# Funatiq/cuclark

Hardware: AMD Instinct MI355X
Metric: Mreads/sec (10M x 150bp, k=31) (higher is better)
Workload: dtype u64

## Files before the change

cuclark_amd/csrc/mic_kernels.hip:

```cpp
#include "mic_internal.h"
#include "mic_device.h"
#include "mic_ksketch.h"
#include "mic_hitmap.h"
#include "mic_join2.h"

#include <stdlib.h>
#include <type_traits>

#ifndef MIC_EXP
#define MIC_EXP 0
#endif
#ifndef MIC_FUNNEL64
#define MIC_FUNNEL64 1
#endif
#ifndef MIC_X
#define MIC_X 0
#endif
#if MIC_X & 8
__device__ unsigned long long g_entry_walk[3];
extern "C" int mic_debug_entry_walk(unsigned long long out[3], int reset) {
  if (hipMemcpyFromSymbol(out, HIP_SYMBOL(g_entry_walk), sizeof(g_entry_walk)) != hipSuccess) return -1;
  const unsigned long long z[3] = {0, 0, 0};
  if (reset && hipMemcpyToSymbol(HIP_SYMBOL(g_entry_walk), z, sizeof(z)) != hipSuccess) return -1;
  return 0;
// ... 931 lines not shown
              bool more0 = v0 && e0 < 6, more1 = v1 && e1 < 6;
              uint32_t hit0 = 0, hit1 = 0;
              e0 = e0 < 5 ? e0 : 5; e1 = e1 < 5 ? e1 : 5;
              for (;;) {
                const uint32_t g0 = q0[e0], g1 = q1[e1];
                const uint32_t a0 = q0[6 + 3 * e0], b0 = q0[7 + 3 * e0], c0 = q0[8 + 3 * e0], p0 = q0[24 + e0];
                const uint32_t a1 = q1[6 + 3 * e1], b1 = q1[7 + 3 * e1], c1 = q1[8 + 3 * e1], p1 = q1[24 + e1];
                const bool same0 = more0 && g0 == t0, same1 = more1 && g1 == t1;
                const bool m0 = same0 && ((p0 >> (16 + (w - 1) - ao[0])) & 1) && s_extract(a0, b0, c0, (int)ao[0], k) == ko[0];
                const bool m1 = same1 && ((p1 >> (16 + (w - 1) - ao[1])) & 1) && s_extract(a1, b1, c1, (int)ao[1], k) == ko[1];
                if (m0) hit0 = (p0 & 0xFFFFu) + 1;
                if (m1) hit1 = (p1 & 0xFFFFu) + 1;
                {
                  const bool cr0 = same0 && (p0 >> 16) == 0, cr1 = same1 && (p1 >> 16) == 0;
                  if (__ballot(cr0) | __ballot(cr1)) {
                    uint64_t kp = (uint64_t)__builtin_amdgcn_kernarg_segment_ptr();
                    asm volatile("" : "+s"(kp));
                    const __attribute__((address_space(4))) MicQueryArgs* kc = (const __attribute__((address_space(4))) MicQueryArgs*)kp;
                    const uint4* side = kc->t.side; const uint32_t smask = kc->t.side_mask;
                    const uint64_t mm = (1ULL << (2 * m)) - 1;
                    if (side && cr0 && s_extract(a0, b0, c0, w - 1, m) == ((ko[0] >> (2 * ao[0])) & mm)) hit0 = s_side_probe(side, smask, ko[0]);
                    if (side && cr1 && s_extract(a1, b1, c1, w - 1, m) == ((ko[1] >> (2 * ao[1])) & mm)) hit1 = s_side_probe(side, smask, ko[1]);
                  }
                }
                more0 = same0 && !m0 && e0 < 5; more1 = same1 && !m1 && e1 < 5;
                e0 += more0 ? 1u : 0u; e1 += more1 ? 1u : 0u;
                if (!(__ballot(more0) | __ballot(more1))) break;
              }
              if (v0) { o0_ = hit0; y0_ = 0xFFFFFFFFu; }
              if (v1) { o1_ = hit1; y1_ = 0xFFFFFFFFu; }
              const bool n0 = v0 && !hit0 && (mz0 & MIC_S_NEXT), n1 = v1 && !hit1 && (mz1 & MIC_S_NEXT);
              if (__ballot(n0) | __ballot(n1)) {
                if (n0 && q0[5] <= t0) y0_ = q0[31];
                if (n1 && q1[5] <= t1) y1_ = q1[31];
              }
            }
          }
        };
        while (__ballot(sl0 != 0xFFFFFFFFu) | __ballot(sl1 != 0xFFFFFFFFu)) {
          uint32_t nx0, nx1;
          level(sl0, sl1, res0, res1, nx0, nx1);
          sl0 = nx0; sl1 = nx1;
        }
        tally2(res0, res1, acc, n_ent, overflow, total, lane);
      }
    }
    uint32_t t_hdr, t_pp, t_pe;
    asm volatile("s_waitcnt vmcnt(0)" ::: "memory");
    __builtin_amdgcn_wave_barrier();
    ahead_take(ahead_sel ? ahead1 : ahead0, n_pp, t_hdr, t_pp, t_pe);
    __builtin_amdgcn_wave_barrier();
    {
      uint64_t kp = (uint64_t)__builtin_amdgcn_kernarg_segment_ptr();
      asm volatile("" : "+s"(kp));
      const __attribute__((address_space(4))) MicQueryArgs* kc = (const __attribute__((address_space(4))) MicQueryArgs*)kp;
      struct { uint32_t* results; uint32_t* rows; uint32_t* flagged; uint32_t row_words, flagged_cap; } fa;
      fa.results = kc->results; fa.rows = kc->rows; fa.flagged = kc->flagged; fa.row_words = kc->row_words; fa.flagged_cap = kc->flagged_cap;
      finish_read(acc, n_ent, total, overflow, r, fa, lane);
    }
    ahead_issue(ahead_sel ? ahead0 : ahead1, t_pp, r + 3 * n_waves);
    ahead_sel ^= 1;
    cur_pp = n_pp; cur_pe = n_pe; cur_hdr = t_hdr; n_pp = t_pp; n_pe = t_pe;
  }
}


__device__ __forceinline__ uint64_t wballot(bool p) { return __builtin_amdgcn_ballot_w64(p); }
#if defined(__has_builtin) && __has_builtin(__builtin_amdgcn_writelane)
__device__ __forceinline__ int mic_writelane(int value, int lane, int old) { return __builtin_amdgcn_writelane(value, lane, old); }
#else
extern "C" __device__ int mic_writelane(int value, int lane, int old) __asm("llvm.amdgcn.writelane.i32");
#endif

static_assert(MIC_RMAX <= 32, "tally_counts sums the first two rows of lanes");
#define MIC_R_CROWDED (-16)
__device__ __forceinline__ void tally_counts(uint32_t lab1, uint32_t cnt, RowAcc& acc, uint32_t& n_ent, uint32_t& overflow,
                                             uint32_t& total, int lane) {
  uint64_t mm = wballot(lab1 != 0);
  while (mm) {
    const uint32_t l1 = __builtin_amdgcn_readlane(lab1, __builtin_ctzll(mm));
    const bool mine = lab1 == l1;
    mm &= ~wballot(mine);
    const uint32_t c = mine ? cnt : 0u;
    uint32_t sum = 0;
    {
      uint32_t v = c;
      v += (uint32_t)__builtin_amdgcn_update_dpp(0, (int)v, 0x111, 0xF, 0xF, true);
      v += (uint32_t)__builtin_amdgcn_update_dpp(0, (int)v, 0x112, 0xF, 0xF, true);
      v += (uint32_t)__builtin_amdgcn_update_dpp(0, (int)v, 0x114, 0xF, 0xF, true);
      v += (uint32_t)__builtin_amdgcn_update_dpp(0, (int)v, 0x118, 0xF, 0xF, true);
      sum = __builtin_amdgcn_readlane(v, 15) + __builtin_amdgcn_readlane(v, 31);
    }
    total += sum;
    if (wballot(acc.label1 == l1)) {
      if (acc.label1 == l1) acc.count += sum;
    } else if (n_ent < 64) {
      acc.label1 = (uint32_t)mic_writelane((int)l1, (int)n_ent, (int)acc.label1);
      acc.count = (uint32_t)mic_writelane((int)sum, (int)n_ent, (int)acc.count);
      ++n_ent;
    } else {
      overflow = 1;
    }
  }
}

template <int KK, int MM, bool FWD, bool PART>
__global__ void __launch_bounds__(64 * MIC_M_WPB, 32 / MIC_M_WPB) query_kernel_r(const MicQueryArgs a) {
  __shared__ uint4 s_stage[MIC_M_WPB][MIC_RMAX * MIC_MSTRIDE + (MIC_RMAX / 8 - 1) * MIC_R_SKEW];
  __shared__ uint16_t s_rec[MIC_M_WPB][132];
  __shared__ uint32_t s_ahead[MIC_M_WPB][2][64];
  __shared__ uint32_t s_part[PART ? MIC_M_WPB : 1][2];
  const int lane = threadIdx.x & 63;
  const int wv = __builtin_amdgcn_readfirstlane(threadIdx.x >> 6);
  uint4* stage = s_stage[wv];
  uint16_t* rec = s_rec[wv];
  const uint32_t wave0 = __builtin_amdgcn_readfirstlane(blockIdx.x * MIC_M_WPB + wv);
  const uint32_t n_waves = gridDim.x * MIC_M_WPB;
  const MicTable& t = a.t;
  if (PART) { if (lane == 0) { s_part[wv][0] = t.slot_lo; s_part[wv][1] = t.slot_cnt; } __builtin_amdgcn_wave_barrier(); }
  const int k = KK ? KK : t.k, m = MM ? MM : t.m, ctx = k - m;
  const uint4* __restrict__ slots = t.slots;
  const uint16_t* __restrict__ cont = a.cont;
  auto below = [](uint64_t mask) { return (uint32_t)__builtin_amdgcn_mbcnt_hi((uint32_t)(mask >> 32), __builtin_amdgcn_mbcnt_lo((uint32_t)mask, 0u)); };

  uint32_t* ahead0 = s_ahead[wv][0];
  uint32_t* ahead1 = s_ahead[wv][1];
  auto lane_copy = [&]() { int ln = lane; asm volatile("" : "+v"(ln)); return ln; };
  auto ahead_issue = [&](uint32_t* entry, uint32_t pp_w, uint32_t r_ptr, const int ln) {
    const uint64_t abase = ((uint64_t)(cont + pp_w)) & ~3ULL;
    const uint32_t rr = r_ptr < a.n_reads ? r_ptr : a.n_reads - 1;
    const uint64_t pbase = (uint64_t)(a.reads_ptr + rr) - 48;
    if (ln < 12)
      __builtin_amdgcn_global_load_lds((const __attribute__((address_space(1))) void*)((const uint32_t*)abase + lane),
                                       (__attribute__((address_space(3))) void*)entry, 4, 0, 0);
    uint64_t pb = pbase + 48;
    asm volatile("" : "+s"(pb));
    if (ln < 2)
      __builtin_amdgcn_global_load_lds((const __attribute__((address_space(1))) void*)((const uint32_t*)pb + lane),
                                       (__attribute__((address_space(3))) void*)(entry + 12), 4, 0, 0);
  };
  auto ahead_take = [&](const uint32_t* entry, uint32_t pp_w, uint32_t& hdr, uint32_t& npp, uint32_t& npe) {
    const uint32_t raw = entry[lane];
    npp = __builtin_amdgcn_readlane(raw, 12); npe = __builtin_amdgcn_readlane(raw, 13);
    const bool odd = (((uint64_t)(cont + pp_w)) >> 1) & 1;
    const uint32_t first = __builtin_amdgcn_readfirstlane(raw);
    hdr = odd ? first >> 16 : first & 0xFFFFu;
  };
  auto ahead_word = [&](const uint32_t* entry, uint32_t pp_w) {
    const uint32_t raw = entry[lane];
    const bool odd = (((uint64_t)(cont + pp_w)) >> 1) & 1;
    const uint32_t up = (uint32_t)__builtin_amdgcn_update_dpp(0, (int)raw, 0x101, 0xF, 0xF, true);
    return __builtin_amdgcn_perm(up, raw, odd ? 0x05040706u : 0x03020504u);
  };
  uint32_t cur_pp, cur_pe, cur_hdr, n_pp, n_pe, ahead_sel;
  {
    const uint32_t r0 = wave0 < a.n_reads ? wave0 : a.n_reads - 1;
    cur_pp = __builtin_amdgcn_readfirstlane(a.reads_ptr[r0]); cur_pe = __builtin_amdgcn_readfirstlane(a.reads_ptr[r0 + 1]);
    ahead_issue(ahead0, cur_pp, wave0 + n_waves, lane_copy());
    asm volatile("s_waitcnt vmcnt(0)" ::: "memory");
    __builtin_amdgcn_wave_barrier();
    ahead_take(ahead0, cur_pp, cur_hdr, n_pp, n_pe);
    ahead_issue(ahead1, n_pp, wave0 + 2 * n_waves, lane_copy());
    ahead_sel = 1;
  }
  constexpr bool PIPE = KK != 0 && (MIC_R_PIPE >= 2 || (MIC_R_PIPE == 1 && FWD));
  struct Round {
    uint32_t G0, G1, G2, cur;
    int jmax, jmin, remaining;
  };
  struct NoGap {};
  struct Gap { uint32_t len1, b2, g0; };
  auto front = [&](const uint32_t first, const uint32_t cend, const uint32_t base, const uint32_t nk, const bool use_ahead, uint32_t& wd_out,
                   const auto gp) __attribute__((always_inline)) -> uint32_t {
    constexpr bool GAP = std::is_same<decltype(gp), const Gap>::value;
    int ln = lane;
    asm volatile("" : "+v"(ln));
    uint32_t wd;
    if constexpr (GAP) {
      const uint32_t* entry = ahead_sel ? ahead0 : ahead1;
      const uint32_t j = (uint32_t)ln < 12u ? (uint32_t)ln : 0u;
      const uint32_t d = j2_dword(j, gp.len1, gp.b2);
      wd = j2_window(ahead_word(entry, cur_pp), entry[d], entry[d + 1u], j, gp.len1, gp.b2);
    } else {
      wd = use_ahead ? ahead_word(ahead_sel ? ahead0 : ahead1, cur_pp)
                     : window_word_w(cont, first, cend, base, ln, false, 0u);
    }
    wd_out = wd;
    const uint32_t n_act = nk - base < 128u ? nk - base : 128u;
    if constexpr (KK == F3_K && MM == F3_M) {
      uint32_t p0, s0, s1, s2, q0, q1, q2;
      if constexpr (GAP) sampled_positions3<!FWD, true>(wd, lane, n_act, p0, s0, s1, s2, q0, q1, q2, gp.len1, gp.g0);
      else sampled_positions3<!FWD>(wd, lane, n_act, p0, s0, s1, s2, q0, q1, q2);
      const uint32_t pv = (uint32_t)__builtin_amdgcn_update_dpp(-1, (int)q2, 0x138, 0xF, 0xF, false);
      const bool f0 = q0 != pv, f1 = q1 != q0, f2 = q2 != q1;
      const uint64_t b0 = wballot(f0), b1 = wballot(f1), b2 = wballot(f2);
      const uint32_t R = __popcll(b0) + __popcll(b1) + __popcll(b2) - 1u;
      uint32_t c = __builtin_amdgcn_mbcnt_hi((uint32_t)(b0 >> 32), __builtin_amdgcn_mbcnt_lo((uint32_t)b0, 0u));
      c = __builtin_amdgcn_mbcnt_hi((uint32_t)(b1 >> 32), __builtin_amdgcn_mbcnt_lo((uint32_t)b1, c));
      c = __builtin_amdgcn_mbcnt_hi((uint32_t)(b2 >> 32), __builtin_amdgcn_mbcnt_lo((uint32_t)b2, c));
      __builtin_amdgcn_wave_barrier();
      const uint32_t c1 = c + (f0 ? 1u : 0u), c2 = c1 + (f1 ? 1u : 0u);
      if (f0) rec[c] = f3_record(s0, p0);
      if (f1) rec[c1] = f3_record(s1, p0 + 1u);
      if (f2) rec[c2] = f3_record(s2, p0 + 2u);
      __builtin_amdgcn_wave_barrier();
      return R;
    }
    const bool past = n_act + (uint32_t)(k - s_tlen(k, m)) >= 129u;
    uint32_t qa0, qa1;
    if constexpr (GAP) sampled_positions<!FWD, true>(wd, ln, lane, k, m, past, qa0, qa1, gp.len1);
    else sampled_positions<!FWD>(wd, ln, lane, k, m, past, qa0, qa1);
    qa0 = (uint32_t)lane < n_act ? qa0 : 0xFFu;
    qa1 = 64u + (uint32_t)lane < n_act ? qa1 : 0xFFu;
    if constexpr (GAP) {
      qa0 = (uint32_t)lane - gp.g0 >= (uint32_t)(k - 1) ? qa0 : 0xFFu;
      qa1 = 64u + (uint32_t)lane - gp.g0 >= (uint32_t)(k - 1) ? qa1 : 0xFFu;
    }
    const uint32_t last0 = __builtin_amdgcn_readlane(qa0, 63);
    uint32_t p0 = (uint32_t)__builtin_amdgcn_update_dpp(-1, (int)qa0, 0x138, 0xF, 0xF, false);
    uint32_t p1 = (uint32_t)__builtin_amdgcn_update_dpp((int)last0, (int)qa1, 0x138, 0xF, 0xF, false);
    const bool f0 = qa0 != p0, f1 = qa1 != p1;
    const uint64_t b0 = wballot(f0), b1 = wballot(f1);
    const uint32_t R0 = __popcll(b0), R = R0 + __popcll(b1) - (n_act < 128u ? 1u : 0u);
    __builtin_amdgcn_wave_barrier();
    if (f0) rec[below(b0)] = (uint16_t)(qa0 | ((uint32_t)lane << 8));
    if (f1) rec[R0 + below(b1)] = (uint16_t)(qa1 | ((64u + (uint32_t)lane) << 8));
    if (__builtin_expect(n_act == 128u, 0)) {
      asm volatile("" ::: "memory");
      if (ln == 0) rec[R] = (uint16_t)(128u << 8);
    }
    __builtin_amdgcn_wave_barrier();
    return R;
  };
  const uint32_t xsh = (64u - 2u * (uint32_t)k) & 31u;
  auto region_x = [&](uint32_t A0, uint32_t A1, uint32_t& lo, uint32_t& hi) {
    if (k > 16) {
      lo = __builtin_amdgcn_alignbit(A0, A1, xsh) & (m >= 16 ? 0xFFFFFFFFu : (1u << ((2 * m) & 31)) - 1u);
      hi = m > 16 ? (A0 >> xsh) & ((1u << ((2 * m - 32) & 31)) - 1u) : 0u;
    } else {
      const uint64_t x = ((((uint64_t)A0 << 32) | A1) << (2 * ctx)) >> (64 - 2 * m);
      lo = (uint32_t)x; hi = (uint32_t)(x >> 32);
    }
  };
  auto setup = [&](const uint32_t wd, const uint32_t rbase, const uint32_t R, Round& L, uint32_t& nrun_out, const auto gp) __attribute__((always_inline)) {
    constexpr bool GAP = std::is_same<decltype(gp), const Gap>::value;
    const uint32_t nrun = R - rbase < MIC_RMAX ? R - rbase : MIC_RMAX;
    nrun_out = nrun;
    bool vr = (uint32_t)lane < nrun;
    const uint32_t ri = vr ? rbase + (uint32_t)lane : 0u;
    const uint32_t rc0 = rec[ri], rc1 = rec[ri + 1];
    const int qa = (int)(rc0 & 255u), i0 = (int)(rc0 >> 8);
    if constexpr (GAP) vr = vr && (uint32_t)i0 != gp.g0;
    const int n = (int)(rc1 >> 8) - i0;
    const int s1 = qa - ctx - 1;
    const int D = s1 >> 4;
    const uint32_t tsh = 30u - 2u * (uint32_t)(s1 & 15);
    const int a0 = D << 2;
    const uint32_t W0 = (uint32_t)__builtin_amdgcn_ds_bpermute(a0, (int)wd), W1 = (uint32_t)__builtin_amdgcn_ds_bpermute(a0 + 4, (int)wd),
                   W2 = (uint32_t)__builtin_amdgcn_ds_bpermute(a0 + 8, (int)wd), W3 = (uint32_t)__builtin_amdgcn_ds_bpermute(a0 + 12, (int)wd);
    uint32_t G0 = __builtin_amdgcn_alignbit(W0, W1, tsh), G1 = __builtin_amdgcn_alignbit(W1, W2, tsh), G2 = __builtin_amdgcn_alignbit(W2, W3, tsh);
    uint32_t key, xhi;
    region_x(G0, G1, key, xhi);
    bool rev = false;
    if (!FWD) {
      const uint32_t sh = 96u - 2u * (uint32_t)(k + ctx);
      const uint32_t r0 = __builtin_bitreverse32(G2), r1 = __builtin_bitreverse32(G1), r2 = __builtin_bitreverse32(G0);
      uint32_t q0, q1, q2;
      if (KK != 0 && sh != 0) {
        q0 = swap_comp_pairs(__builtin_amdgcn_alignbit(r0, r1, 33u - sh), __builtin_amdgcn_alignbit(r0, r1, 31u - sh));
        q1 = swap_comp_pairs(__builtin_amdgcn_alignbit(r1, r2, 33u - sh), __builtin_amdgcn_alignbit(r1, r2, 31u - sh));
        q2 = swap_comp_pairs(r2 << (sh - 1u), r2 << (sh + 1u));
      } else {
        q0 = sh ? __builtin_amdgcn_alignbit(r0, r1, 32u - sh) : r0;
        q1 = sh ? __builtin_amdgcn_alignbit(r1, r2, 32u - sh) : r1;
        q2 = r2 << sh;
        q0 = swap_comp_pairs(q0 >> 1, q0 << 1); q1 = swap_comp_pairs(q1 >> 1, q1 << 1); q2 = swap_comp_pairs(q2 >> 1, q2 << 1);
      }
      uint32_t kr, hr;
      region_x(q0, q1, kr, hr);
      rev = hr < xhi || (hr == xhi && kr < key);
      G0 = rev ? q0 : G0; G1 = rev ? q1 : G1; G2 = rev ? q2 : G2;
      key = rev ? kr : key; xhi = rev ? hr : xhi;
    }
    const int jmaxf = qa - i0, jminf = jmaxf - n + 1;
    const int jmax = rev ? ctx - jminf : jmaxf, jmin = rev ? ctx - jmaxf : jminf;
    uint32_t cur = vr ? sslot_of_x32(key, xhi, (uint32_t)t.n_main) : 0xFFFFFFFFu;
    bool mine = vr;
    if (PART) {
      mine = vr && cur - s_part[wv][0] < s_part[wv][1];
      cur = mine ? cur : 0xFFFFFFFFu;
    }
    L.G0 = G0; L.G1 = G1; L.G2 = G2; L.cur = cur;
    L.jmax = jmax; L.jmin = jmin; L.remaining = mine ? n : 0;
  };
  auto issue = [&](const uint32_t cur, const uint32_t nrun, const int ln) __attribute__((always_inline)) {
    uint32_t sidx[MIC_RMAX / 8];
    __builtin_amdgcn_wave_barrier();
    if (ln < MIC_RMAX) ((uint32_t*)stage)[lane] = cur;
    __builtin_amdgcn_wave_barrier();
    uint32_t so = (uint32_t)(uintptr_t)(__attribute__((address_space(3))) void*)stage;
    asm volatile("" : "+s"(so));
#pragma unroll
    for (int i = 0; i < MIC_RMAX / 8; ++i) sidx[i] = ((const uint32_t*)stage)[8 * i + (lane >> 3)];
#pragma unroll
    for (int i = 0; i < MIC_RMAX / 8; ++i) {
      if (8u * i >= nrun) break;
      if (sidx[i] != 0xFFFFFFFFu)
        __builtin_amdgcn_global_load_lds((const __attribute__((address_space(1))) void*)(slots + (uint64_t)sidx[i] * 8 + (lane & 7)),
                                         (__attribute__((address_space(3))) void*)(uintptr_t)(so + 16u * (64 + MIC_R_SKEW) * (uint32_t)i), 16, 0, 0);
    }
  };
  auto consume = [&](Round& L, RowAcc& acc, uint32_t& n_ent, uint32_t& overflow, uint32_t& total, uint32_t& cg) __attribute__((always_inline)) {
    const uint32_t G0 = L.G0, G1 = L.G1, G2 = L.G2;
    uint32_t key, xhi_;
    region_x(G0, G1, key, xhi_);
    const int jmax = L.jmax, jmin = L.jmin;
    uint32_t cur = L.cur;
    int remaining = L.remaining;
    for (;;) {
      asm volatile("s_waitcnt vmcnt(0)" ::: "memory");
      __builtin_amdgcn_wave_barrier();
      const bool vl = cur != 0xFFFFFFFFu;
      const uint32_t* q = (const uint32_t*)(stage + (vl ? staged_at((uint32_t)lane) : 0));
      const uint4 ka = *(const uint4*)q;
      const uint2 kb = *(const uint2*)(q + 4);
      uint32_t e = (ka.x < key) + (ka.y < key) + (ka.z < key) + (ka.w < key) + (kb.x < key) + (kb.y < key);
      const uint32_t mz = q[30];
      const uint64_t m_vl = wballot(vl);
      uint64_t m_more = m_vl & wballot(e < 6), m_pos = 0;
      e = e < 5 ? e : 5;
#if MIC_X & 8
      uint32_t ew_pass = 0;
#endif
      for (;;) {
        uint32_t e3 = e + (e << 1);
        asm volatile("" : "+v"(e3));
        uint32_t g = q[e], g1 = q[e + 1], S0 = q[6 + e3], S1 = q[7 + e3], S2 = q[8 + e3], pl = q[24 + e];
        asm volatile("" : "+v"(S2));
        const uint64_t m_same = m_more & wballot(g == key);
        const uint64_t m_next = wballot(g1 == key);
        const uint32_t d0 = G0 ^ S0, d1 = G1 ^ S1, d2 = G2 ^ S2;
        const uint64_t m_hit = m_same & (k > 16
                                             ? wballot(((d0 & ((1u << ((32 - 2 * ctx) & 31)) - 1u)) | (d1 >> xsh)) == 0)
                                             : wballot((((((uint64_t)d0 << 32) | d1) << (2 * ctx)) >> (64 - 2 * m)) == 0));
        const uint32_t dl = d0 >> (32 - 2 * ctx);
        const uint32_t dr = k > 16 ? __builtin_amdgcn_alignbit(d1, d2, xsh)
                                        : (uint32_t)((((((uint64_t)d0 << 32) | d1)) << ((2 * k) & 63)) >> 32);
        const int left = __builtin_ctz(dl | (1u << (2 * ctx))) >> 1;
        const int right = __builtin_clz(dr | (1u << (31 - 2 * ctx))) >> 1;
        const int hi = left < jmax ? left : jmax, lo = ctx - right > jmin ? ctx - right : jmin;
        const uint32_t range = ((2u << (hi & 31)) - 1u) & (~0u << (lo & 31));
        const uint32_t hits = __builtin_amdgcn_inverse_ballot_w64(m_hit) ? (uint32_t)__popc((pl >> 16) & range) : 0u;
#if MIC_X & 8
        const bool ew_hit = wballot(hits != 0) != 0;
        if (lane == 0 && ew_pass < 2u) atomicAdd(&g_entry_walk[ew_pass], 1ull);
        if (lane == 0 && ew_pass == 1u && ew_hit) atomicAdd(&g_entry_walk[2], 1ull);
        ++ew_pass;
#endif
        const uint32_t lab_new = (pl & 0xFFFFu) + 1u;
#if !(MIC_X & 16)
        tally_counts(hits ? lab_new : 0u, hits, acc, n_ent, overflow, total, lane);
#endif
#if MIC_X & 32
        break;
#endif
#if !(MIC_X & 1)
        remaining = __builtin_amdgcn_inverse_ballot_w64(m_hit & wballot(pl < 0x10000u)) ? MIC_R_CROWDED : remaining;
#endif
        remaining -= (int)hits;
        m_pos = wballot(remaining > 0);
        m_more = m_same & m_pos & wballot(e < 5);
#if !(MIC_X & 256)
        m_more &= m_next;
#endif
        e += __builtin_amdgcn_inverse_ballot_w64(m_more) ? 1u : 0u;
        if (!m_more) break;
      }
#if MIC_X & 64
      break;
#endif
      const uint64_t m_nx = m_pos & wballot((mz & MIC_S_NEXT) != 0);
      if (!m_nx) break;
      cur = 0xFFFFFFFFu;
      if (__builtin_amdgcn_inverse_ballot_w64(m_nx) && q[5] <= key) cur = q[31];
      if (!wballot(cur != 0xFFFFFFFFu)) break;
      remaining = (cur == 0xFFFFFFFFu && remaining > 0) ? 0 : remaining;
      issue(cur, MIC_RMAX, lane_copy());
    }
    if (!(MIC_X & 2) && __builtin_expect(wballot(remaining <= MIC_R_CROWDED) != 0, 0)) {
      const bool crowded = remaining <= MIC_R_CROWDED;
      const uint32_t n_c = (uint32_t)__popcll(wballot(crowded));
      uint64_t kpv = (uint64_t)__builtin_amdgcn_kernarg_segment_ptr();
      asm volatile("" : "+v"(kpv));
      const MicQueryArgs* kv = (const MicQueryArgs*)kpv;
      uint32_t* cw = kv->crowd;
      uint32_t* itb = kv->crowd_items;
      const uint32_t icap = kv->crowd_item_cap;
      uint32_t ib = 0xFFFFFFFFu;
      if (cw != nullptr && cg != MIC_CG_DENSE) {
        uint32_t v = 0;
        if (lane == 0) v = atomicAdd(&cw[1], n_c);
        ib = __builtin_amdgcn_readfirstlane(v);
      }
      asm volatile("" : "+v"(ib));
      const bool room = ib <= icap && n_c <= icap - ib;
      if (crowded && room) {
        uint32_t* it = itb + 8 * ((size_t)ib + below(wballot(crowded)));
        it[0] = G0; it[1] = G1; it[2] = G2; it[3] = (uint32_t)jmin | ((uint32_t)jmax << 8);
        it[4] = cg;
      }
      cg = __builtin_amdgcn_readfirstlane(room ? (ib | ((n_c - 1u) << 27)) : MIC_CG_DENSE);
    }
  };
  auto finish = [&](const RowAcc& acc, uint32_t n_ent, uint32_t total, uint32_t overflow, uint32_t r, const uint32_t cg) __attribute__((always_inline)) {
    uint32_t spilled = 0;
    if (!(MIC_X & 4) && __builtin_expect(cg != MIC_CG_NONE, 0)) {
      uint64_t kpv = (uint64_t)__builtin_amdgcn_kernarg_segment_ptr();
      asm volatile("" : "+v"(kpv));
      const MicQueryArgs* kv = (const MicQueryArgs*)kpv;
      uint32_t* cw = kv->crowd;
      uint32_t* pool = kv->crowd_pool;
      const uint32_t pcap = kv->crowd_pend_cap, wcap = kv->crowd_pool_cap;
      uint32_t p = 0xFFFFFFFFu, off = 0;
      if (cg != MIC_CG_DENSE) {
        if (lane == 0) { p = atomicAdd(&cw[0], 1u); off = atomicAdd(&cw[2], 2u * n_ent); }
        p = __builtin_amdgcn_readfirstlane(p); off = __builtin_amdgcn_readfirstlane(off);
      }
      asm volatile("" : "+v"(p), "+v"(off));
      const bool room = off <= wcap && 2u * n_ent <= wcap - off;
      if (p < pcap) {
        uint32_t* pd = cw + MIC_CROWD_HDR + 8 * (size_t)p;
        if (lane == 0) { pd[0] = r; pd[1] = total; pd[2] = room ? (n_ent | (overflow << 8)) : 0xFFFFFFFFu; pd[3] = off; pd[4] = cg; }
        if (room && (uint32_t)lane < n_ent) { uint32_t* pe_ = pool + (size_t)off + 2 * lane; pe_[0] = acc.label1; pe_[1] = acc.count; }
      }
      spilled = __builtin_amdgcn_readfirstlane((p < pcap && room) ? 1u : 0u);
      if (!spilled) {
        if (lane == 0 && cw != nullptr && cg != MIC_CG_DENSE) atomicAdd(&cw[3], 1u);
        overflow = 1;
      }
    }
    if (!spilled) {
      uint64_t kp = (uint64_t)__builtin_amdgcn_kernarg_segment_ptr();
      asm volatile("" : "+s"(kp));
      const __attribute__((address_space(4))) MicQueryArgs* kc = (const __attribute__((address_space(4))) MicQueryArgs*)kp;
      struct { uint32_t* results; uint32_t* rows; uint32_t* flagged; uint32_t row_words, flagged_cap; } fa;
      fa.results = kc->results; fa.rows = kc->rows; fa.flagged = kc->flagged; fa.row_words = kc->row_words; fa.flagged_cap = kc->flagged_cap;
      finish_read(acc, n_ent, total, overflow, r, fa, lane);
    }
  };

  uint32_t r = wave0; bool p_valid = false;
  auto step = [&](Round& P, Round& N) __attribute__((always_inline)) -> bool {
    const bool have = r < a.n_reads;
    uint32_t pp = cur_pp;
    const uint32_t pe = cur_pe;
    bool shape = false, simple = false;
    uint32_t n_nrun = 0, plen0 = 0, pp1 = 0;
    uint32_t slot2 = J2_NONE;
    if (have) {
      plen0 = cur_hdr; pp1 = pp + 1 + (plen0 + 7) / 8;
      shape = plen0 - (uint32_t)k < 128u && pp1 == pe;
      if (!shape && plen0 - (uint32_t)k < 128u && pp1 < pe) {
        const uint32_t rel = pp1 - cur_pp + (uint32_t)((((uint64_t)(cont + cur_pp)) >> 1) & 1);
        if (rel < 24u) {
          const uint32_t v = (ahead_sel ? ahead0 : ahead1)[rel >> 1];
          slot2 = __builtin_amdgcn_readfirstlane((rel & 1u) ? v >> 16 : v & 0xFFFFu);
          shape = slot2 == 0;
        }
      }
      uint32_t n_wd = 0, R = MIC_RMAX + 1u, g0 = 0xFFFFFFFFu;
      if (PIPE && shape) {
        R = front(pp + 1, pp1, 0u, plen0 - (uint32_t)k + 1u, true, n_wd, NoGap{});
      } else if constexpr (PIPE) {
        const uint32_t odd = (uint32_t)((((uint64_t)(cont + cur_pp)) >> 1) & 1);
        const uint32_t* entry = ahead_sel ? ahead0 : ahead1;
        const J2Shape j2 = j2_shape(plen0, slot2, pe - pp, odd, (uint32_t)k,
                                    [&](uint32_t u) { return (uint32_t)__builtin_amdgcn_readfirstlane(j2_half(entry[u >> 1], u)); });
        if (__builtin_expect(j2.ok != 0u, 0)) {
          R = front(pp + 1, pp1, 0u, j2.n_act, true, n_wd, Gap{j2.len1, j2.b2, j2.g0});
          g0 = j2.g0;
        }
      }
      if (PIPE && R <= MIC_RMAX) { setup(n_wd, 0u, R, N, n_nrun, Gap{0u, 0u, g0}); simple = true; }
    }
    if (PIPE && p_valid) {
      RowAcc acc; acc.label1 = 0; acc.count = 0;
      uint32_t n_ent = 0, overflow = 0, total = 0, cg = MIC_CG_NONE;
      consume(P, acc, n_ent, overflow, total, cg);
      finish(acc, n_ent, total, overflow, r - n_waves, cg);
    } else {
      asm volatile("s_waitcnt vmcnt(0)" ::: "memory");
    }
    if (!have) return false;
    if (!simple) {
      RowAcc acc; acc.label1 = 0; acc.count = 0;
      uint32_t n_ent = 0, overflow = 0, total = 0, cg = MIC_CG_NONE;
      auto chunk = [&](const uint32_t first, const uint32_t cend, const uint32_t base, const uint32_t nk, const bool use_ahead) __attribute__((always_inline)) {
        uint32_t wd;
        const uint32_t R = front(first, cend, base, nk, use_ahead, wd, NoGap{});
        for (uint32_t rbase = 0; rbase < R; rbase += MIC_RMAX) {
          Round L; uint32_t nrun;
          setup(wd, rbase, R, L, nrun, NoGap{});
          issue(L.cur, nrun, lane_copy());
          consume(L, acc, n_ent, overflow, total, cg);
        }
      };
      if (!PIPE && shape) chunk(pp + 1, pp1, 0u, plen0 - (uint32_t)k + 1u, true);
      else {
        bool first_part = true;
        while (pp < pe) {
          uint32_t plen;
          {
            const uint32_t rel = pp - cur_pp + (uint32_t)((((uint64_t)(cont + cur_pp)) >> 1) & 1);
            if (first_part) plen = cur_hdr;
            else if (rel < 24u) {
              const uint32_t v = (ahead_sel ? ahead0 : ahead1)[rel >> 1];
              plen = __builtin_amdgcn_readfirstlane((rel & 1u) ? v >> 16 : v & 0xFFFFu);
            } else plen = __builtin_amdgcn_readfirstlane((uint32_t)cont[pp]);
          }
          const bool ahead_ok = first_part;
          first_part = false;
          if (plen == 0) break;
          const uint32_t first = pp + 1;
          pp = first + (plen + 7) / 8;
          if (plen < (uint32_t)k) continue;
          const uint32_t nk = plen - k + 1;
          const uint32_t cend = pp;
          for (uint32_t base = 0; base < nk; base += 128) chunk(first, cend, base, nk, ahead_ok && base == 0);
        }
      }
      finish(acc, n_ent, total, overflow, r, cg);
    }
    uint32_t t_hdr, t_pp, t_pe;
    __builtin_amdgcn_wave_barrier();
    ahead_take(ahead_sel ? ahead1 : ahead0, n_pp, t_hdr, t_pp, t_pe);
    __builtin_amdgcn_wave_barrier();
    const int ln = lane_copy();
    ahead_issue(ahead_sel ? ahead0 : ahead1, t_pp, r + 3 * n_waves, ln);
    ahead_sel ^= 1;
    cur_pp = n_pp; cur_pe = n_pe; cur_hdr = t_hdr; n_pp = t_pp; n_pe = t_pe;
    p_valid = simple;
    if (simple) issue(N.cur, n_nrun, ln);
    r += n_waves;
    return true;
  };
  Round Ra, Rb;
  while (step(Ra, Rb) && step(Rb, Ra)) {}
}

__global__ void __launch_bounds__(256) crowd_finish_kernel(const MicQueryArgs a) {
  const int lane = threadIdx.x & 63;
  const uint32_t wave0 = __builtin_amdgcn_readfirstlane(blockIdx.x * 4 + (threadIdx.x >> 6)), n_waves = gridDim.x * 4;
  const uint32_t* __restrict__ cw = a.crowd;
  const uint32_t pcap = a.crowd_pend_cap;
  uint32_t np = cw[0];
  np = np < pcap ? np : pcap;
  const uint32_t* __restrict__ pend = cw + MIC_CROWD_HDR;
  const uint32_t* __restrict__ items = a.crowd_items;
  const uint32_t* __restrict__ pool = a.crowd_pool;
  const uint4* __restrict__ side = a.t.side;
  const uint32_t smask = a.t.side_mask;
  const int k = a.t.k, ctx = k - a.t.m;
  for (uint32_t p = wave0; p < np; p += n_waves) {
    const uint4 h = *(const uint4*)(pend + 8 * (size_t)p);
    const uint32_t r = __builtin_amdgcn_readfirstlane(h.x), meta = __builtin_amdgcn_readfirstlane(h.z), off = __builtin_amdgcn_readfirstlane(h.w);
    uint32_t total = __builtin_amdgcn_readfirstlane(h.y);
    uint32_t g = __builtin_amdgcn_readfirstlane(pend[8 * (size_t)p + 4]);
    if (meta == 0xFFFFFFFFu) continue;
    uint32_t n_ent = meta & 0xFFu, overflow = (meta >> 8) & 1u;
    RowAcc acc; acc.label1 = 0; acc.count = 0;
    if ((uint32_t)lane < n_ent) { const uint2 e = *(const uint2*)(pool + off + 2 * lane); acc.label1 = e.x; acc.count = e.y; }
    while (g != MIC_CG_NONE) {
      const uint32_t ib = g & 0x7FFFFFFu, n_c = (g >> 27) + 1u;
      g = __builtin_amdgcn_readfirstlane(items[8 * (size_t)ib + 4]);
      for (uint32_t b = 0; b < n_c; b += 4) {
        const uint32_t idx = b + ((uint32_t)lane >> 4);
        const bool valid = idx < n_c;
        uint4 it = make_uint4(0, 0, 0, 0);
        if (valid) it = *(const uint4*)(items + 8 * (size_t)(ib + idx));
        const int jmin = (int)(it.w & 0xFFu), jmax = (int)((it.w >> 8) & 0xFFu);
        int j = jmin + (lane & 15);
        bool go = valid && j <= jmax;
        j = go ? j : jmin;
        const uint64_t K = s_extract(it.x, it.y, it.z, ctx - j, k);
        uint32_t hsh = s_side_hash(K, smask), got = 0;
        while (wballot(go)) {
          uint4 c = make_uint4(0, 0, 0, 0);
          if (go) c = load_slot_quarter(side + hsh);
          if (go) {
            if (c.z == 0) go = false;
            else if (c.x == (uint32_t)K && c.y == (uint32_t)(K >> 32)) { got = c.z; go = false; }
            else hsh = (hsh + 1) & smask;
          }
        }
        tally2(got, 0u, acc, n_ent, overflow, total, lane);
      }
    }
    finish_read(acc, n_ent, total, overflow, r, a, lane);
  }
}


__global__ void merge_rows_kernel(const uint32_t* __restrict__ ra, const uint32_t* __restrict__ rb,
                                  uint32_t* __restrict__ out, uint32_t row_words, size_t n,
                                  uint32_t* __restrict__ results) {
  size_t i = (size_t)blockIdx.x * blockDim.x + threadIdx.x;
  if (i >= n) return;
  const uint32_t* a = ra + i * row_words; const uint32_t* b = rb + i * row_words; uint32_t* o = out + i * row_words;
  uint32_t na = a[0], nb = b[0], ia = 0, ib = 0, no = 0;
  bool ok = na != MIC_ROW_INVALID && nb != MIC_ROW_INVALID;
  if (!ok) { na = 0; nb = 0; }
  while (ia < na || ib < nb) {
    uint32_t va = ia < na ? a[1 + ia] : 0xFFFFFFFFu, vb = ib < nb ? b[1 + ib] : 0xFFFFFFFFu;
    uint32_t ta = ia < na ? (va & 0xFFFF) : 0x10000u, tb = ib < nb ? (vb & 0xFFFF) : 0x10000u;
    uint32_t tgt, cnt;
    if (ta < tb) { tgt = ta; cnt = va >> 16; ++ia; }
    else if (tb < ta) { tgt = tb; cnt = vb >> 16; ++ib; }
    else { tgt = ta; cnt = (va >> 16) + (vb >> 16); ++ia; ++ib; }
    if (no + 1 < row_words && cnt <= 0xFFFF) o[1 + no] = (cnt << 16) | tgt; else ok = false;
    ++no;
  }
  o[0] = ok ? no : MIC_ROW_INVALID;
  (void)results;
}

__global__ void result_rows_kernel(const uint32_t* __restrict__ rows, uint32_t row_words,
                                   uint32_t* __restrict__ results, size_t n) {
  size_t i = (size_t)blockIdx.x * blockDim.x + threadIdx.x;
  if (i >= n) return;
  const uint32_t* row = rows + i * row_words;
  uint32_t cnt = row[0], sum = 0, best = 0, ib = 0, sb = 0, is = 0, flags = 0;
  if (cnt == MIC_ROW_INVALID) { cnt = 0; flags = MIC_FLAG_ROW_OVERFLOW_; }
  for (uint32_t e = 0; e < cnt; ++e) {
    uint32_t v = row[1 + e], tgt = v & 0xFFFF, sc = v >> 16;
    if (sc > best) { sb = best; is = ib; best = sc; ib = tgt + 1; }
    else if (sc > sb) { sb = sc; is = tgt + 1; }
    sum += sc;
  }
  uint4* out = (uint4*)(results + i * 8);
  out[0] = make_uint4(sum, ib, best, is);
  out[1] = make_uint4(sb, cnt, flags, 0);
}

template <bool KEY64>
__device__ inline uint32_t probe_scalar(const MicTable& t, uint64_t kmer) {
  constexpr uint32_t CAP = KEY64 ? MIC_CAP64 : MIC_CAP32;
  uint64_t c = canonical(kmer, t.k);
  uint64_t q = mic_div(c, t.div);
  uint64_t rem = c - q * t.div.d;
  if (rem < t.shard_start || rem >= t.shard_end) return 0;
  if (!KEY64 && (q >> 32) != 0) return 0;
  uint64_t slot = rem - t.shard_start;
  for (;;) {
    uint4 qq[4];
#pragma unroll
    for (int j = 0; j < 4; ++j) qq[j] = t.slots[slot * 4 + j];
    uint32_t n = qq[0].w & 0xFF;
    uint64_t lastk = 0;
#pragma unroll
    for (int j = 0; j < 4; ++j) {
      uint32_t m = match_quarter<KEY64>(qq[j], (uint32_t)q, (uint32_t)(q >> 32), j);
      if (m) return m;
    }
    lastk = KEY64 ? (((uint64_t)qq[3].y << 32) | qq[3].x) : (uint64_t)qq[3].y;
    if (n <= CAP || q <= lastk) return 0;
    slot = (uint64_t)(qq[0].w >> 8) | ((uint64_t)(qq[1].w >> 8) << 24);
  }
}

__device__ inline uint32_t probe_scalar_m(const MicTable& t, uint64_t kmer) {
  uint64_t c = canonical(kmer, t.k);
  if (t.sharded) {
    uint64_t q = mic_div(c, t.div);
    uint64_t rem = c - q * t.div.d;
    if (rem < t.shard_start || rem >= t.shard_end) return 0;
  }
  uint64_t slot = mslot_of_kmer(kmer, t.k, t.m, (uint32_t)t.n_main);
  for (;;) {
    const uint4* q = t.slots + slot * 8;
    const uint4 meta = q[7];
    const uint32_t n = MIC_M_N(meta.z);
    uint32_t cnt = 0;
    bool eq = false;
    for (uint32_t e = 0; e < n; ++e) {
      uint4 kv = q[e >> 1];
      uint64_t key = (e & 1) ? (((uint64_t)kv.w << 32) | kv.z) : (((uint64_t)kv.y << 32) | kv.x);
      if (key <= c) { ++cnt; eq = key == c; }
    }
    if (!(meta.z & MIC_M_DIR)) {
      if (!eq) return 0;
      const uint32_t e = cnt - 1;
      uint4 lw = q[6 + (e >> 3)];
      uint32_t wi = (e & 7) >> 1;
      uint32_t word = wi == 0 ? lw.x : wi == 1 ? lw.y : wi == 2 ? lw.z : lw.w;
      return ((e & 1) ? (word >> 16) : (word & 0xFFFF)) + 1;
    }
    if (cnt == 0) return 0;
    slot = (uint64_t)q[6].x + (cnt - 1);
  }
}
// ... 452 lines not shown
```

Before: 2285.

## Restructure read pipeline loop into steady-state fast path with fallback road

Replaces the single generic step lambda, which carried have/simple/p_valid flags every iteration, with a split control flow. A steady-state loop alternates the take_up/back_half/issue halves while reads stay simple, and falls back to a plain per-read path when they do not. The ahead-buffer selection flag becomes swapped pointers (e_cur/e_nxt) instead of ternaries on each access. The goal is to cut scalar branching and selects in the hot loop and to let the compiler schedule the pipelined path more tightly. It adds code size and more complex loop exits, which risks register pressure or a missed final drain.

Result: faster. 2323 (median of 6 runs) (+1.7%).

```diff
diff --git a/cuclark_amd/csrc/mic_kernels.hip b/cuclark_amd/csrc/mic_kernels.hip
--- a/cuclark_amd/csrc/mic_kernels.hip
+++ b/cuclark_amd/csrc/mic_kernels.hip
@@ -1107,7 +1107,7 @@
     const uint32_t up = (uint32_t)__builtin_amdgcn_update_dpp(0, (int)raw, 0x101, 0xF, 0xF, true);
     return __builtin_amdgcn_perm(up, raw, odd ? 0x05040706u : 0x03020504u);
   };
-  uint32_t cur_pp, cur_pe, cur_hdr, n_pp, n_pe, ahead_sel;
+  uint32_t cur_pp, cur_pe, cur_hdr, n_pp, n_pe;
   {
     const uint32_t r0 = wave0 < a.n_reads ? wave0 : a.n_reads - 1;
     cur_pp = __builtin_amdgcn_readfirstlane(a.reads_ptr[r0]); cur_pe = __builtin_amdgcn_readfirstlane(a.reads_ptr[r0 + 1]);
@@ -1116,8 +1116,8 @@
     __builtin_amdgcn_wave_barrier();
     ahead_take(ahead0, cur_pp, cur_hdr, n_pp, n_pe);
     ahead_issue(ahead1, n_pp, wave0 + 2 * n_waves, lane_copy());
-    ahead_sel = 1;
-  }
+  }
+  uint32_t *e_cur = ahead0, *e_nxt = ahead1;
   constexpr bool PIPE = KK != 0 && (MIC_R_PIPE >= 2 || (MIC_R_PIPE == 1 && FWD));
   struct Round {
     uint32_t G0, G1, G2, cur;
@@ -1132,12 +1132,12 @@
     asm volatile("" : "+v"(ln));
     uint32_t wd;
     if constexpr (GAP) {
-      const uint32_t* entry = ahead_sel ? ahead0 : ahead1;
+      const uint32_t* entry = e_cur;
       const uint32_t j = (uint32_t)ln < 12u ? (uint32_t)ln : 0u;
       const uint32_t d = j2_dword(j, gp.len1, gp.b2);
       wd = j2_window(ahead_word(entry, cur_pp), entry[d], entry[d + 1u], j, gp.len1, gp.b2);
     } else {
-      wd = use_ahead ? ahead_word(ahead_sel ? ahead0 : ahead1, cur_pp)
+      wd = use_ahead ? ahead_word(e_cur, cur_pp)
                      : window_word_w(cont, first, cend, base, ln, false, 0u);
     }
     wd_out = wd;
@@ -1404,31 +1404,90 @@
     }
   };
 
-  uint32_t r = wave0; bool p_valid = false;
-  auto step = [&](Round& P, Round& N) __attribute__((always_inline)) -> bool {
-    const bool have = r < a.n_reads;
+  uint32_t r = wave0;
+  auto plain_road = [&]() __attribute__((always_inline)) {
     uint32_t pp = cur_pp;
     const uint32_t pe = cur_pe;
-    bool shape = false, simple = false;
-    uint32_t n_nrun = 0, plen0 = 0, pp1 = 0;
-    uint32_t slot2 = J2_NONE;
-    if (have) {
-      plen0 = cur_hdr; pp1 = pp + 1 + (plen0 + 7) / 8;
-      shape = plen0 - (uint32_t)k < 128u && pp1 == pe;
-      if (!shape && plen0 - (uint32_t)k < 128u && pp1 < pe) {
-        const uint32_t rel = pp1 - cur_pp + (uint32_t)((((uint64_t)(cont + cur_pp)) >> 1) & 1);
-        if (rel < 24u) {
-          const uint32_t v = (ahead_sel ? ahead0 : ahead1)[rel >> 1];
-          slot2 = __builtin_amdgcn_readfirstlane((rel & 1u) ? v >> 16 : v & 0xFFFFu);
-          shape = slot2 == 0;
+    RowAcc acc; acc.label1 = 0; acc.count = 0;
+    uint32_t n_ent = 0, overflow = 0, total = 0, cg = MIC_CG_NONE;
+    auto chunk = [&](const uint32_t first, const uint32_t cend, const uint32_t base, const uint32_t nk, const bool use_ahead) __attribute__((always_inline)) {
+      uint32_t wd;
+      const uint32_t R = front(first, cend, base, nk, use_ahead, wd, NoGap{});
+      for (uint32_t rbase = 0; rbase < R; rbase += MIC_RMAX) {
+        Round L; uint32_t nrun;
+        setup(wd, rbase, R, L, nrun, NoGap{});
+        issue(L.cur, nrun, lane_copy());
+        consume(L, acc, n_ent, overflow, total, cg);
+      }
+    };
+    const uint32_t plen0 = cur_hdr, pp1 = pp + 1 + (plen0 + 7) / 8;
+    if (!PIPE && plen0 - (uint32_t)k < 128u && pp1 == pe) chunk(pp + 1, pp1, 0u, plen0 - (uint32_t)k + 1u, true);
+    else {
+      bool first_part = true;
+      while (pp < pe) {
+        uint32_t plen;
+        {
+          const uint32_t rel = pp - cur_pp + (uint32_t)((((uint64_t)(cont + cur_pp)) >> 1) & 1);
+          if (first_part) plen = cur_hdr;
+          else if (rel < 24u) {
+            const uint32_t v = e_cur[rel >> 1];
+            plen = __builtin_amdgcn_readfirstlane((rel & 1u) ? v >> 16 : v & 0xFFFFu);
+          } else plen = __builtin_amdgcn_readfirstlane((uint32_t)cont[pp]);
+        }
+        const bool ahead_ok = first_part;
+        first_part = false;
+        if (plen == 0) break;
+        const uint32_t first = pp + 1;
+        pp = first + (plen + 7) / 8;
+        if (plen < (uint32_t)k) continue;
+        const uint32_t nk = plen - k + 1;
+        const uint32_t cend = pp;
+        for (uint32_t base = 0; base < nk; base += 128) chunk(first, cend, base, nk, ahead_ok && base == 0);
+      }
+    }
+    finish(acc, n_ent, total, overflow, r, cg);
+  };
+  auto advance = [&]() __attribute__((always_inline)) -> int {
+    uint32_t t_hdr, t_pp, t_pe;
+    __builtin_amdgcn_wave_barrier();
+    ahead_take(e_nxt, n_pp, t_hdr, t_pp, t_pe);
+    __builtin_amdgcn_wave_barrier();
+    const int ln = lane_copy();
+    ahead_issue(e_cur, t_pp, r + 3 * n_waves, ln);
+    { uint32_t* const e = e_cur; e_cur = e_nxt; e_nxt = e; }
+    cur_pp = n_pp; cur_pe = n_pe; cur_hdr = t_hdr; n_pp = t_pp; n_pe = t_pe;
+    r += n_waves;
+    return ln;
+  };
+  if constexpr (!PIPE) {
+    while (r < a.n_reads) {
+      asm volatile("s_waitcnt vmcnt(0)" ::: "memory");
+      plain_road();
+      advance();
+    }
+  } else {
+    auto take_up = [&](Round& N) __attribute__((always_inline)) -> uint32_t {
+      const uint32_t pp = cur_pp, pe = cur_pe;
+      const uint32_t plen0 = cur_hdr, pp1 = pp + 1 + (plen0 + 7) / 8;
+      bool shape = false;
+      uint32_t slot2 = J2_NONE;
+      if (__builtin_expect(plen0 - (uint32_t)k < 128u, 1)) {
+        if (__builtin_expect(pp1 == pe, 1)) shape = true;
+        else if (pp1 < pe) {
+          const uint32_t rel = pp1 - cur_pp + (uint32_t)((((uint64_t)(cont + cur_pp)) >> 1) & 1);
+          if (rel < 24u) {
+            const uint32_t v = e_cur[rel >> 1];
+            slot2 = __builtin_amdgcn_readfirstlane((rel & 1u) ? v >> 16 : v & 0xFFFFu);
+            shape = slot2 == 0;
+          }
         }
       }
       uint32_t n_wd = 0, R = MIC_RMAX + 1u, g0 = 0xFFFFFFFFu;
-      if (PIPE && shape) {
+      if (shape) {
         R = front(pp + 1, pp1, 0u, plen0 - (uint32_t)k + 1u, true, n_wd, NoGap{});
-      } else if constexpr (PIPE) {
+      } else {
         const uint32_t odd = (uint32_t)((((uint64_t)(cont + cur_pp)) >> 1) & 1);
-        const uint32_t* entry = ahead_sel ? ahead0 : ahead1;
+        const uint32_t* entry = e_cur;
         const J2Shape j2 = j2_shape(plen0, slot2, pe - pp, odd, (uint32_t)k,
                                     [&](uint32_t u) { return (uint32_t)__builtin_amdgcn_readfirstlane(j2_half(entry[u >> 1], u)); });
         if (__builtin_expect(j2.ok != 0u, 0)) {
@@ -1436,71 +1495,49 @@
           g0 = j2.g0;
         }
       }
-      if (PIPE && R <= MIC_RMAX) { setup(n_wd, 0u, R, N, n_nrun, Gap{0u, 0u, g0}); simple = true; }
-    }
-    if (PIPE && p_valid) {
+      if (R <= MIC_RMAX) { uint32_t nrun; setup(n_wd, 0u, R, N, nrun, Gap{0u, 0u, g0}); }
+      else R = MIC_RMAX + 1u;
+      return R;
+    };
+    auto back_half = [&](Round& P) __attribute__((always_inline)) {
       RowAcc acc; acc.label1 = 0; acc.count = 0;
       uint32_t n_ent = 0, overflow = 0, total = 0, cg = MIC_CG_NONE;
       consume(P, acc, n_ent, overflow, total, cg);
       finish(acc, n_ent, total, overflow, r - n_waves, cg);
-    } else {
+    };
+    auto half_in = [&](Round& P, Round& N) __attribute__((always_inline)) -> uint32_t {
+      uint32_t R = MIC_RMAX + 1u;
+      if (r < a.n_reads) R = take_up(N);
+      asm volatile("" : "+s"(R));
+      back_half(P);
+      return R;
+    };
+    auto half_out = [&](Round& N, const uint32_t R) __attribute__((always_inline)) {
+      const int ln = advance();
+      issue(N.cur, R, ln);
+    };
+    Round Ra, Rb;
+    while (r < a.n_reads) {
+      const uint32_t R = take_up(Ra);
       asm volatile("s_waitcnt vmcnt(0)" ::: "memory");
-    }
-    if (!have) return false;
-    if (!simple) {
-      RowAcc acc; acc.label1 = 0; acc.count = 0;
-      uint32_t n_ent = 0, overflow = 0, total = 0, cg = MIC_CG_NONE;
-      auto chunk = [&](const uint32_t first, const uint32_t cend, const uint32_t base, const uint32_t nk, const bool use_ahead) __attribute__((always_inline)) {
-        uint32_t wd;
-        const uint32_t R = front(first, cend, base, nk, use_ahead, wd, NoGap{});
-        for (uint32_t rbase = 0; rbase < R; rbase += MIC_RMAX) {
-          Round L; uint32_t nrun;
-          setup(wd, rbase, R, L, nrun, NoGap{});
-          issue(L.cur, nrun, lane_copy());
-          consume(L, acc, n_ent, overflow, total, cg);
+      if (R <= MIC_RMAX) {
+        const int ln = advance();
+        issue(Ra.cur, R, ln);
+        for (;;) {
+          const uint32_t Rn = half_in(Ra, Rb);
+          if (Rn > MIC_RMAX) break;
+          half_out(Rb, Rn);
+          const uint32_t Rm = half_in(Rb, Ra);
+          if (Rm > MIC_RMAX) break;
+          half_out(Ra, Rm);
         }
-      };
-      if (!PIPE && shape) chunk(pp + 1, pp1, 0u, plen0 - (uint32_t)k + 1u, true);
-      else {
-        bool first_part = true;
-        while (pp < pe) {
-          uint32_t plen;
-          {
-            const uint32_t rel = pp - cur_pp + (uint32_t)((((uint64_t)(cont + cur_pp)) >> 1) & 1);
-            if (first_part) plen = cur_hdr;
-            else if (rel < 24u) {
-              const uint32_t v = (ahead_sel ? ahead0 : ahead1)[rel >> 1];
-              plen = __builtin_amdgcn_readfirstlane((rel & 1u) ? v >> 16 : v & 0xFFFFu);
-            } else plen = __builtin_amdgcn_readfirstlane((uint32_t)cont[pp]);
-          }
-          const bool ahead_ok = first_part;
-          first_part = false;
-          if (plen == 0) break;
-          const uint32_t first = pp + 1;
-          pp = first + (plen + 7) / 8;
-          if (plen < (uint32_t)k) continue;
-          const uint32_t nk = plen - k + 1;
-          const uint32_t cend = pp;
-          for (uint32_t base = 0; base < nk; base += 128) chunk(first, cend, base, nk, ahead_ok && base == 0);
-        }
+        if (!(r < a.n_reads)) break;
       }
-      finish(acc, n_ent, total, overflow, r, cg);
-    }
-    uint32_t t_hdr, t_pp, t_pe;
-    __builtin_amdgcn_wave_barrier();
-    ahead_take(ahead_sel ? ahead1 : ahead0, n_pp, t_hdr, t_pp, t_pe);
-    __builtin_amdgcn_wave_barrier();
-    const int ln = lane_copy();
-    ahead_issue(ahead_sel ? ahead0 : ahead1, t_pp, r + 3 * n_waves, ln);
-    ahead_sel ^= 1;
-    cur_pp = n_pp; cur_pe = n_pe; cur_hdr = t_hdr; n_pp = t_pp; n_pe = t_pe;
-    p_valid = simple;
-    if (simple) issue(N.cur, n_nrun, ln);
-    r += n_waves;
-    return true;
-  };
-  Round Ra, Rb;
-  while (step(Ra, Rb) && step(Rb, Ra)) {}
+      plain_road();
+      advance();
+    }
+  }
+  asm volatile("s_waitcnt vmcnt(0)" ::: "memory");
 }
 
 __global__ void __launch_bounds__(256) crowd_finish_kernel(const MicQueryArgs a) {
```
